# pkmtum/generative-physics-informed-pde

Measured on AMD Instinct MI355X. Metric: ELBO training-step samples/sec (64x64 grids), higher is better.
Workload: dtype f32; 1 GPU; BASELINE config 2/3: c64 grid, B_u=256 unlabeled + N_s=32 labeled per GPU, ROM 8x8, fused native step; global_batch=288, grid=64, parallelism=dp1, graph=True, graph_mode=streams, steps_per_replay=4, world=1, bn=replica

## Files before the change

generative-physics-informed-pde_amd/csrc/conv.hip:

```cpp
#include "common.h"
#include <stdlib.h>
#include <stdio.h>
#include <algorithm>
#include <string.h>
#include <string>
#include <type_traits>
#include <utility>
#include <vector>
#include <atomic>
#include <mutex>

using namespace gpi;

#pragma clang fp contract(on)

namespace {

constexpr int HALO = 4;

__device__ __attribute__((aligned(256))) float g_zero_page[64];

struct Div {
    uint32_t m, one;
};
// ... 1168 lines not shown
__host__ __device__ inline bool vop_op(const gpi_conv_desc& d) {
    return d.k == 5 && d.stride == 1 && !d.upsample && d.gin_off >= 0 && d.cin <= 4 && d.cout <= 2;
}
__host__ __device__ inline int bwd_rowlen(const gpi_conv_desc& d) {
    return d.cout * d.cin * d.k * d.k + (d.in_bn ? 2 * d.cin : 0);
}
__host__ __device__ inline int vop_mid_floats(int gh, int w_out, int rowlen, bool fuse);
template <bool B>
struct BoolC {
    static constexpr bool value = B;
};

template <int V>
struct IntC {
    static constexpr int value = V;
};

constexpr int GPI_BWD_WAVES = 6;
constexpr int SLAB_ROWS = 4;
__host__ __device__ inline int vop_mid_floats(int gh, int w_out, int rowlen, bool fuse) {
    return pad256(512 + SLAB_ROWS * rowlen);
}

constexpr int GPI_FUSE_WAVES = 5;
constexpr int GPI_FUSE_SHP_WAVES = 5;

template <typename T>
__device__ __forceinline__ T splat(float v);
template <>
__device__ __forceinline__ float splat<float>(float v) { return v; }
template <>
__device__ __forceinline__ f32x2 splat<f32x2>(float v) { return f32x2{v, v}; }

template <int K, int S, int UP, bool FUSE = false, bool HALF = false, int EXF = 0, int SHP = -1>
__global__ __launch_bounds__(256) __attribute__((amdgpu_waves_per_eu(K == 5 ? (FUSE ? (SHP >= 0 ? GPI_FUSE_SHP_WAVES : GPI_FUSE_WAVES) : 4) : GPI_BWD_WAVES))) void conv_bwd_kernel(gpi_conv_desc d, gpi_codec_ctx c, ConvGeom G) {
    fold_shape<SHP>(d, G);
    touch_kernargs<CONV_KARG_BYTES>();
    entry_signal(G);
    if (SKIP(G, 16)) return;
    ConvGeom Gt_;
    if constexpr (HALF) {
        const int lb0 = logical_block(G);
        const bool wgr0 = G.split && (G.xcd ? (lb0 & 1) != 0 : lb0 >= G.nblocks);
        const int tile0 = !G.split ? lb0 : (G.xcd ? lb0 >> 1 : (wgr0 ? lb0 - G.nblocks : lb0));
        Gt_ = G;
        if (tile0 >= G.nfull) set_half_tile(Gt_);
    }
    const ConvGeom& Gt = HALF ? Gt_ : G;
    constexpr int KK = K * K;
    extern __shared__ __attribute__((aligned(16))) float smem[];
    double* gst = (double*)smem;
    float* i_sc = smem + 8 * (d.cin + d.cout);
    float* i_sh = i_sc + d.cin;
    float* i_mean = i_sh + d.cin;
    float* i_inv = i_mean + d.cin;
    float* i_gam = i_inv + d.cin;
    float* o_coef = i_gam + d.cin;
    float* o_drop = o_coef + 4 * d.cout;
    const bool has_gin = d.gin_off >= 0;
    const bool obn = d.gout_mode == 0;
    const int KD = d.cout * KK;
    const int KD4 = (KD + 3) & ~3;
    const bool vop = FUSE || (K == 5 && S == 1 && !UP && has_gin && d.cin <= 4 && d.cout <= 2);
    const int J = d.cin * KK;
    const int rowlen = d.cout * J + (d.in_bn ? 2 * d.cin : 0);
    float* wD = smem + bwd_hdr(d.cin, d.cout);
    const int nwd = (has_gin && !vop) ? KD4 * 16 : 0;
    float* const mid = wD;
// ... 284 lines not shown
        constexpr bool bern = EXF == 2;
        using acc_t = std::conditional_t<bern, float, f32x2>;
        const float scl = karg_sel(c.loss_scale, T.grp);
        const float xlo = bern ? karg_sel(c.tgt_lo, T.grp) : 0.f;
        const int nrg = (Gt.gh + RPF - 1) / RPF, nitem = nrg * d.w_out;
        auto fwd_items = [&](auto ci_c) {
            constexpr int CIN = decltype(ci_c)::value;
            for (int it = tid; it < nitem; it += 256) {
                const int rg = dq(it, Gt.d_wout), x = it - rg * d.w_out;
                const int j0 = rg * RPF;
                float tv[bern ? 1 : RPF];
                uint32_t tb = tb0;
                if constexpr (bern) {
                    if (it != tid) {
                        tb = 0;
#pragma unroll
                        for (int p = 0; p < RPF; ++p) {
                            const int oy = gy0 + j0 + p;
                            const bool ok = j0 + p < Gt.gh && oy >= 0 && oy < d.h_out;
                            tb |= ((ok ? as_gld(tg)[oy * d.w_out + x] : 0.f) != xlo ? 1u : 0u) << p;
                        }
                    }
                } else {
#pragma unroll
                    for (int p = 0; p < RPF; ++p) {
                        const int oy = gy0 + j0 + p;
                        const bool ok = j0 + p < Gt.gh && oy >= 0 && oy < d.h_out;
                        tv[p] = it == tid ? tv0[p] : (ok ? as_gld(tg)[oy * d.w_out + x] : 0.f);
                    }
                }
                acc_t acc[RPF];
#pragma unroll
                for (int p = 0; p < RPF; ++p) acc[p] = splat<acc_t>(0.f);
#pragma unroll(bern ? 1 : CIN)
                for (int ci = 0; ci < CIN; ++ci) {
                    if (ci >= d.cin) break;
                    const float* acol = al + ci * Gt.rh * Gt.P + HALO + x - PADK;
#pragma unroll(bern ? 1 : K)
                    for (int kx = 0; kx < K; ++kx) {
                        float v[RPF + K - 1];
#pragma unroll
                        for (int r = 0; r < RPF + K - 1; ++r) v[r] = acol[min(j0 + r, Gt.rh - 1) * Gt.P + kx];
                        acc_t w[K];
#pragma unroll
                        for (int ky = 0; ky < K; ++ky) {
                            const int i = ((ci * K + kx) * K + ky) * NCO;
                            w[ky] = *reinterpret_cast<const acc_t*>(mid + 256 + i);
                        }
#pragma unroll
                        for (int r = 0; r < RPF + K - 1; ++r) {
#pragma unroll
                            for (int p = 0; p < RPF; ++p) {
                                const int ky = r - p;
                                if (ky < 0 || ky >= K) continue;
                                acc[p] = __builtin_elementwise_fma(w[ky], splat<acc_t>(v[r]), acc[p]);
                            }
                        }
                    }
                }
#pragma unroll
                for (int p = 0; p < RPF; ++p) {
                    const int j = j0 + p, oy = gy0 + j;
                    if (j >= Gt.gh || oy < 0 || oy >= d.h_out) continue;
                    const bool own = j >= PADK && j < PADK + Gt.th;
                    float* g0 = gl + j * Gt.PG + HALO + x;
                    if constexpr (bern) {
                        float ll, gv;
// ... 224 lines not shown
                                const int co2 = i2 / K, kx2 = i2 - co2 * K;
                                if (ucls) {
                                    const int ci2 = j2 >> 1, rr = j2 & 1, py = (T.oy0 + wv) & 1;
                                    const int kyl = rr ? 1 + py : 0, kyh = rr ? 2 : py;
                                    float* const sp = slab + co2 * J + ci2 * KK + kx2;
                                    sp[kyl * K] = acc[u][r];
                                    if (kyh != kyl) sp[kyh * K] = acc[u][r];
                                } else {
                                    const int ci2 = j2 / K, ky2 = j2 - ci2 * K;
                                    slab[co2 * J + ci2 * KK + ky2 * K + kx2] = acc[u][r];
                                }
                            }
                        }
                    }
                }
            }
        }
    };
    const int bsel = Gt.alt == 1 ? (int)(blockIdx.x >> 8) : Gt.alt == 2 ? (int)(blockIdx.x >> 3) : (int)blockIdx.x;
    const bool wg_late = FUSE && Gt.alt != 0 && (bsel & 1) != 0;
    if (vop && !wg_late) wgrad_phase();
    PHASE(5);

    float sd = 0.f, sdx = 0.f;
    if (nmblk > 0) {
        float l_bet = 0.f, l_rgam = 0.f, l_gam = 0.f;
        if (d.in_bn) {
            l_gam = i_gam[ci_l];
            l_bet = i_sh[ci_l] + i_mean[ci_l] * i_sc[ci_l];
            l_rgam = 1.f / l_gam;
        }
        const float* arow0 = alb + (ci_l * Gt.rh + (py0 - iy0)) * Gt.P + HALO;
        const int nkd = KD4 >> 2;
        for (int round = 0; wv + 16 * round < nmblk; ++round) {
            if (round > 0 && S != 2) own_load(round, pv4);
#pragma unroll
            for (int u = 0; u < 4; ++u) {
                const int m = wv + 4 * (4 * round + u);
                if (m < nmblk) {
                    const int i = 16 * m + l16;
                    const int qy = dq(i, Gt.d_win), px = i - qy * d.w_in;
                    f32x4 acc = {0.f, 0.f, 0.f, 0.f};
                    if (S == 2) {
                        const int nbc = nmblk >> 2, cls = m / nbc, mb = m - cls * nbc;
                        const int ry = cls >> 1, rx = cls & 1;
                        const int nky = (K - ((ry + d.pad) & 1) + 1) >> 1, nkx = (K - ((rx + d.pad) & 1) + 1) >> 1;
                        const int nk = __builtin_amdgcn_readfirstlane(d.cout * nky * nkx);
                        const int cp = 16 * mb + l16, a2 = dq(cp, Gt.d_w2), b2 = cp - a2 * (d.w_in >> 1);
                        const float* ab = gl + ((py0 >> 1) - gy0 + a2) * Gt.PG + b2 + HALO;
                        const int2* tAB = reinterpret_cast<const int2*>(ktab + cls * 2 * KD4);
                        const int nks = (nk + 3) >> 2;
                        int ks = 0;
                        for (; ks + 4 <= nks; ks += 4) {
                            int2 t[4];
                            float a[4], b[4];
#pragma unroll
                            for (int u = 0; u < 4; ++u) t[u] = tAB[4 * (ks + u) + kq];
#pragma unroll
                            for (int u = 0; u < 4; ++u) {
                                a[u] = ab[t[u].x];
                                b[u] = wD[t[u].y + l16];
                            }
#pragma unroll
                            for (int u = 0; u < 4; ++u) acc = mfma4(4 * (ks + u) + kq < nk ? a[u] : 0.f, b[u], acc);
                        }
                        for (; ks < nks; ++ks) {
// ... 278 lines not shown

size_t bwd_lds(const gpi_conv_desc& d, const ConvGeom& G) {
    return sizeof(float) * bwd_lds_floats(d, G.rh, G.P, G.gh, G.PG, G.zreg, G.fuse != 0);
}

bool lsum_op(const gpi_conv_desc& d, const ConvGeom& G) {
    static const int on = env_int("GPI_LSUM", 2);
    if (!on || vop_op(d) || G.fuse) return false;
    if ((on == 2 && d.h_out * d.w_out > 256) || (on == 3 && d.h_out * d.w_out > 64)) return false;
    if (d.k == 7 && d.stride == 2 && !d.upsample && d.cin == 1 && d.gin_off < 0 && d.cout <= 16) return false;
    if (d.cout * d.k > 32 || d.cin * d.k > 32) return false;
    const size_t avail = bwd_lds_floats(d, G.rh, G.P, G.gh, G.PG, G.zreg, false) - bwd_hdr(d.cin, d.cout);
    return avail >= (size_t)4 * bwd_rowlen(d);
}

bool vsum_op(const gpi_conv_desc& d, const ConvGeom& G) {
    static const int on = env_int("GPI_VSUM", 1);
    if (!on || !(d.k == 7 && d.stride == 2 && !d.upsample && d.cin == 1 && d.gin_off < 0 && d.cout <= 16)) return false;
    return (size_t)img_floats(d.cout, G.gh, G.PG) >= (size_t)4 * bwd_rowlen(d);
}

typedef void (*conv_kernel_t)(gpi_conv_desc, gpi_codec_ctx, ConvGeom);

#ifndef GPI_CONV_SHAPE_NOFOLD
#define GPI_CONV_SHAPE_NOFOLD {-1}
#endif
constexpr int kNoFold[] = GPI_CONV_SHAPE_NOFOLD;
constexpr bool no_fold(int i) {
    for (int v : kNoFold)
        if (v == i) return true;
    return false;
}

template <int I>
conv_kernel_t shape_kernel() {
    constexpr ShapeC s = kShapes[I];
    if constexpr (no_fold(I)) return nullptr;
    else if constexpr (s.fwd != 0) return conv_fwd_kernel<s.D_k, s.D_stride, s.D_upsample, s.cp, s.npxk, s.half != 0, I>;
    else return conv_bwd_kernel<s.D_k, s.D_stride, s.upk, s.fusek != 0, s.half != 0, s.exf, I>;
}

template <int LO, int... I>
conv_kernel_t shape_kernel_at(int i, std::integer_sequence<int, I...>) {
    static const conv_kernel_t t[] = {shape_kernel<LO + I>()..., nullptr};
    return t[i];
}

}

namespace gpi_conv_parts {
__attribute__((visibility("hidden"))) void* shape_part1(int i);
__attribute__((visibility("hidden"))) void* shape_part2(int i);
__attribute__((visibility("hidden"))) void* shape_part3(int i);
#if GPI_CONV_SHAPE_PART > 0
#define GPI_PART_FN_(p) shape_part##p
#define GPI_PART_FN(p) GPI_PART_FN_(p)
void* GPI_PART_FN(GPI_CONV_SHAPE_PART)(int i) {
    constexpr int lo = kBounds[GPI_CONV_SHAPE_PART], n = kBounds[GPI_CONV_SHAPE_PART + 1] - lo;
    return (void*)shape_kernel_at<lo>(i, std::make_integer_sequence<int, n>{});
}
#endif
}

namespace {
#if GPI_CONV_SHAPE_PART == 0

template <int K, int S, int UP, int NPX, bool HALF>
conv_kernel_t pick_cp_h(int cp) {
    if (cp == 2) return conv_fwd_kernel<K, S, UP, 2, NPX, HALF>;
    if (cp == 4) return conv_fwd_kernel<K, S, UP, 4, NPX, HALF>;
    if (cp == 6) return conv_fwd_kernel<K, S, UP, 6, NPX, HALF>;
    return conv_fwd_kernel<K, S, UP, 8, NPX, HALF>;
}

template <int K, int S, int UP, int NPX>
conv_kernel_t pick_cp(int cp, bool half = false) {
    if constexpr (NPX != 0) {
        if (half) return pick_cp_h<K, S, UP, NPX, true>(cp);
    }
    return pick_cp_h<K, S, UP, NPX, false>(cp);
}

template <int K, int S, int UP>
conv_kernel_t pick(int cp, bool fwd, int npx, bool half, bool ucls = false) {
    if constexpr (UP != 0) {
        if (!fwd && ucls) return half ? conv_bwd_kernel<K, S, 2, false, true> : conv_bwd_kernel<K, S, 2>;
    }
    if (!fwd) return half ? conv_bwd_kernel<K, S, UP, false, true> : conv_bwd_kernel<K, S, UP>;
    if constexpr (K == 3 && S == 1) {
        if (npx == NPX_ROWS2) {
            if (cp == 4) return half ? conv_fwd_kernel<K, S, UP, 4, NPX_ROWS2, true> : conv_fwd_kernel<K, S, UP, 4, NPX_ROWS2>;
            if (cp == 6) return half ? conv_fwd_kernel<K, S, UP, 6, NPX_ROWS2, true> : conv_fwd_kernel<K, S, UP, 6, NPX_ROWS2>;
            return half ? conv_fwd_kernel<K, S, UP, 8, NPX_ROWS2, true> : conv_fwd_kernel<K, S, UP, 8, NPX_ROWS2>;
        }
    }
// ... 59 lines not shown
    s.wout = d.wpart_off >= 0;
    s.ext_in = d.in_off < 0;
    if (fuse) {
        s.half = half;
        s.exf = exf;
        s.upk = 0;
    } else if (!fwd) {
        s.half = half;
        s.upk = (d.upsample && G.ucls) ? 2 : d.upsample;
    } else {
        const int npx = G.cg > 1 ? 0 : G.npx;
        s.npxk = (npx == 0 && !(d.upsample == 0 && d.k <= 3)) ? 1 : npx;
        s.half = s.npxk == 0 ? 0 : half;
        s.cp = cp;
    }
#define F(n) s.D_##n = d.n;
    SHAPE_D(F)
#undef F
#define F(n) s.G_##n = G.n;
    SHAPE_G(F)
#undef F
#define F(n) s.M_##n = (int)G.n.m, s.O_##n = (int)G.n.one;
    SHAPE_GD(F)
#undef F
#define F(n) s.A_##n = G.ha.n;
    SHAPE_A(F)
#undef F
#define F(n) s.AM_##n = (int)G.ha.n.m, s.AO_##n = (int)G.ha.n.one;
    SHAPE_AD(F)
#undef F
    return s;
}

conv_kernel_t shape_kernel_any(int i) {
    if (i < 0 || i >= kNumShapes) return nullptr;
    if (i < kBounds[1]) return shape_kernel_at<0>(i, std::make_integer_sequence<int, kBounds[1]>{});
    if (i < kBounds[2]) return (conv_kernel_t)gpi_conv_parts::shape_part1(i - kBounds[1]);
    if (i < kBounds[3]) return (conv_kernel_t)gpi_conv_parts::shape_part2(i - kBounds[2]);
    return (conv_kernel_t)gpi_conv_parts::shape_part3(i - kBounds[3]);
}

std::atomic<int64_t> g_shape_planned{0}, g_shape_matched{0};
std::vector<ShapeC> g_shapes_seen;
std::mutex g_shapes_mu;

int shape_index(const ShapeC& s) {
    for (int i = 0; i < kNumShapes; ++i)
        if (memcmp(&kShapes[i], &s, sizeof(ShapeC)) == 0) return i;
    return -1;
}

int launch(const gpi_conv_desc& d, const gpi_codec_ctx& c, hipStream_t st, bool fwd, bool fuse = false,
           uint32_t* sig = nullptr, const int64_t* sig_epoch = nullptr, bool dry = false) {
    ConvGeom G;
    if (!conv_geom(d, c.groups, G, fwd, fuse)) return GPI_ERR_UNSUPPORTED;
    if (sig && !sig_epoch) return GPI_ERR_ARG;
    G.sig = sig;
    G.sig_epoch = sig_epoch;
    const bool bern = d.epilogue == GPI_EPI_BERNOULLI_LOSS;
    if (bern && (d.cout != 1 || d.gout_mode != 1)) return GPI_ERR_ARG;
    if (bern && (d.k != 5 || d.stride != 1 || d.upsample)) return GPI_ERR_UNSUPPORTED;
    if (bern && (fwd || fuse) && !dry)
        for (int g = 0; g < c.groups.n_groups; ++g)
            if (!c.tgt[g]) return GPI_ERR_ARG;
    if (fuse && (fwd || d.k != 5 || d.stride != 1 || d.upsample || d.cout != (bern ? 1 : 2) || d.cin > 4 ||
                 d.drop_off >= 0 || d.gout_mode != 1 || d.gin_off < 0 || !loss_epi(d.epilogue)))
        return GPI_ERR_UNSUPPORTED;
    if (gauss_epi(d.epilogue) && d.cout != 2) return GPI_ERR_ARG;
    if (d.in_off < 0 && !c.ext_in) return GPI_ERR_ARG;
    if (!aligned_ok(d, c, fwd)) return GPI_ERR_UNSUPPORTED;
    if (!fwd && d.gin_off >= 0 && ((G.ph * d.w_in) & 15)) return GPI_ERR_UNSUPPORTED;
    if (!fwd && d.gin_off >= 0 && d.stride == 2 && ((d.w_in & 7) || (G.ph & 1))) return GPI_ERR_UNSUPPORTED;
    const int cp = cp_of(d);
    const int exf = bern ? 2 : d.epilogue == GPI_EPI_GAUSS_EXP_LOSS ? 1 : 0;
    conv_kernel_t k = select_kernel(d, cp, fwd, G.cg > 1 ? 0 : G.npx, G.nfull < G.nblocks, G.ucls != 0, fuse, exf);
    if (!k) return GPI_ERR_UNSUPPORTED;
    static const float* zero = nullptr;
    if (!zero && !dry) {
        void* p = nullptr;
        if (hipGetSymbolAddress(&p, HIP_SYMBOL(g_zero_page)) != hipSuccess) return GPI_ERR_LAUNCH;
        zero = (const float*)p;
    }
    G.zero = zero;
    if (!fwd) G.lsum = lsum_op(d, G) ? 1 : 0;
    if (!fwd) G.vsum = vsum_op(d, G) ? 1 : 0;
    const size_t lds = fwd ? fwd_lds(d, G, cp) : bwd_lds(d, G);
    if (lds > 160 * 1024) return GPI_ERR_UNSUPPORTED;
    if (!fwd && d.gin_off >= 0 && !fuse && !vop_op(d)) {
        static const int split_env = env_int("GPI_BWD_SPLIT", 1);
        const int per_cu = std::min((int)(160000 / std::max<size_t>(lds, 1)), d.k == 5 ? 4 : 6);
        G.split = (split_env && d.wpart_off >= 0 && 2 * G.nblocks <= std::min(per_cu, 4) * 256) ? 1 : 0;
    }
    const int grid = G.nblocks * (G.split ? 2 : 1);
    G.grid = grid;
    G.xcd = xcd_mode(fwd, fuse, G.split != 0, G.nfull < G.nblocks) ? 1 : 0;
    static const int fuse_alt = env_int("GPI_FUSE_ALT", 1);
    G.alt = fuse ? fuse_alt : 0;
    {
        const int shapes_on = env_int("GPI_CONV_SHAPES", 1);
        static const int record = env_int("GPI_CONV_SHAPES_RECORD", 0);
        const ShapeC s = shape_of(d, G, fwd, fuse, cp, exf);
        g_shape_planned += dry ? 0 : 1;
        const int si = shapes_on ? shape_index(s) : -1;
        const conv_kernel_t ks = si >= 0 ? shape_kernel_any(si) : nullptr;
        if (ks) {
            k = ks;
            g_shape_matched += dry ? 0 : 1;
        }
        if (record || dry) {
            std::lock_guard<std::mutex> lk(g_shapes_mu);
            bool seen = false;
            for (const ShapeC& q : g_shapes_seen) seen = seen || memcmp(&q, &s, sizeof(ShapeC)) == 0;
            if (!seen) g_shapes_seen.push_back(s);
        }
        if (dry) return GPI_OK;
    }
#ifdef GPI_PHASE_TIMING
    static const int dbg_print = env_int("GPI_DBG_PRINT", 0);
    if (dbg_print)
        fprintf(stderr, "conv %s k%d s%d up%d cin%d cout%d in%dx%d out%dx%d th%d blocks %d lds %zu\n",
                fwd ? "fwd" : "bwd", d.k, d.stride, d.upsample, d.cin, d.cout, d.h_in, d.w_in, d.h_out, d.w_out, G.th,
                G.nblocks, lds);
#endif
    if (lds > 64 * 1024) {
        if (hipFuncSetAttribute((const void*)k, hipFuncAttributeMaxDynamicSharedMemorySize, (int)lds) != hipSuccess)
            return GPI_ERR_LAUNCH;
    }
    hipLaunchKernelGGL(k, dim3(grid), dim3(256), lds, st, d, c, G);
    GPI_CHECK_LAUNCH();
    return GPI_OK;
}

#ifndef GPI_RROWS
#define GPI_RROWS 64
#endif
constexpr int RROWS = GPI_RROWS;

// ... 80 lines not shown
    const int threads = n_items * max_channels;
    hipLaunchKernelGGL(bn_running_kernel, dim3((threads + 255) / 256), dim3(256), 0, (hipStream_t)stream, items, n_items,
                       max_channels, stats, n_stats, momentum);
    GPI_CHECK_LAUNCH();
    return GPI_OK;
}

constexpr uint32_t PROBE_SENTINEL = 0xdeadbeefu;
__global__ __launch_bounds__(64) void buffer_lds_probe_kernel(const float* src, int bytes, const int32_t* off16,
                                                              const int32_t* off4, uint32_t* out) {
    __shared__ __attribute__((aligned(16))) float lds[320];
    const int lane = threadIdx.x;
    for (int i = lane; i < 320; i += 64) lds[i] = __builtin_bit_cast(float, PROBE_SENTINEL);
    __syncthreads();
    const rsrc_t rs = make_rsrc(src, bytes);
    blds16(rs, off16[lane], lds);
    blds4(rs, off4[lane], lds + 256);
    asm volatile("s_waitcnt vmcnt(0)" ::: "memory");
    __syncthreads();
    for (int i = lane; i < 320; i += 64) out[i] = __builtin_bit_cast(uint32_t, lds[i]);
}

extern "C" int gpi_debug_buffer_lds_probe(const float* src, int32_t bytes, const int32_t* off16, const int32_t* off4,
                                          uint32_t* out, void* stream) {
    if (!src || !off16 || !off4 || !out || bytes <= 0 || (bytes & 15) || ((uintptr_t)src & 15)) return GPI_ERR_ARG;
    hipLaunchKernelGGL(buffer_lds_probe_kernel, dim3(1), dim3(64), 0, (hipStream_t)stream, src, (int)bytes, off16, off4,
                       out);
    GPI_CHECK_LAUNCH();
    return GPI_OK;
}

#ifdef GPI_PHASE_TIMING
extern "C" int gpi_debug_phase_stamps(unsigned long long* phase, unsigned long long* rt) {
    static unsigned long long zeros[4096 * 16];
    if (hipMemcpyFromSymbol(phase, HIP_SYMBOL(g_phase), sizeof(zeros)) != hipSuccess) return GPI_ERR_LAUNCH;
    if (hipMemcpyFromSymbol(rt, HIP_SYMBOL(g_rt), sizeof(unsigned long long) * 4096 * 2) != hipSuccess)
        return GPI_ERR_LAUNCH;
    if (hipMemcpyToSymbol(HIP_SYMBOL(g_phase), zeros, sizeof(zeros)) != hipSuccess) return GPI_ERR_LAUNCH;
    if (hipMemcpyToSymbol(HIP_SYMBOL(g_rt), zeros, sizeof(unsigned long long) * 4096 * 2) != hipSuccess)
        return GPI_ERR_LAUNCH;
    return GPI_OK;
}
#endif

extern "C" int gpi_conv_blocks(const gpi_conv_desc* op, const gpi_groups* groups, int32_t* blocks) {
    if (!op || !groups || !blocks) return GPI_ERR_ARG;
    ConvGeom G;
    if (!conv_geom(*op, *groups, G, false)) return GPI_ERR_UNSUPPORTED;
    *blocks = G.nblocks * ((vop_op(*op) || lsum_op(*op, G) || vsum_op(*op, G)) ? 1 : SLAB_ROWS);
    return GPI_OK;
}

extern "C" int gpi_conv_launch_info(const gpi_conv_desc* op, const gpi_groups* groups, int fwd, int32_t* info) {
    if (!op || !groups || !info) return GPI_ERR_ARG;
    ConvGeom G;
    if (!conv_geom(*op, *groups, G, fwd != 0)) return GPI_ERR_UNSUPPORTED;
    const int cp = cp_of(*op);
    info[0] = G.th;
    info[1] = G.nblocks;
    info[2] = (int32_t)(fwd ? fwd_lds(*op, G, cp) : bwd_lds(*op, G));
    info[3] = cp;
    info[4] = G.npx;
    info[5] = G.P;
    info[6] = G.PG;
    return GPI_OK;
}

extern "C" int gpi_conv_shape_info(int64_t* info) {
    if (!info) return GPI_ERR_ARG;
    info[0] = kNumShapes;
    info[1] = g_shape_planned;
    info[2] = g_shape_matched;
    {
        std::lock_guard<std::mutex> lk(g_shapes_mu);
        info[3] = (int64_t)g_shapes_seen.size();
    }
    return GPI_OK;
}

extern "C" int gpi_conv_shape_plan(const gpi_conv_desc* op, const gpi_codec_ctx* ctx, int fwd, int fuse) {
    if (!op || !ctx) return GPI_ERR_ARG;
    return launch(*op, *ctx, nullptr, fwd != 0, fuse != 0, nullptr, nullptr, true);
}

extern "C" int gpi_conv_shapes_dump(char* buf, int64_t len) {
    if (!buf || len <= 0) return GPI_ERR_ARG;
    std::lock_guard<std::mutex> lk(g_shapes_mu);
    std::string out = "#define GPI_CONV_SHAPE_COUNT " + std::to_string(g_shapes_seen.size()) + "\n#define GPI_CONV_SHAPE_LIST";
    for (const ShapeC& s : g_shapes_seen) {
        const int* f = reinterpret_cast<const int*>(&s);
        out += " \\\n    {";
        for (size_t i = 0; i < sizeof(ShapeC) / sizeof(int); ++i) out += (i ? "," : "") + std::to_string(f[i]);
        out += "},";
    }
    out += "\n";
    if ((int64_t)out.size() + 1 > len) return GPI_ERR_ARG;
    memcpy(buf, out.c_str(), out.size() + 1);
    return GPI_OK;
}

extern "C" int gpi_conv_forward(const gpi_conv_desc* op, const gpi_codec_ctx* ctx, void* stream) {
    if (!op || !ctx) return GPI_ERR_ARG;
    return launch(*op, *ctx, (hipStream_t)stream, true);
}

extern "C" int gpi_conv_backward(const gpi_conv_desc* op, const gpi_codec_ctx* ctx, void* stream) {
    if (!op || !ctx) return GPI_ERR_ARG;
    return launch(*op, *ctx, (hipStream_t)stream, false);
}

// ... 73 lines not shown
```

generative-physics-informed-pde_amd/gpi/_lib.py:

```python
import ctypes as C
import os

import torch

HERE = os.path.dirname(os.path.abspath(__file__))
LIB_PATH = os.path.join(HERE, 'libgpi_hip.so')
if os.environ.get('GPI_LIB_VARIANT'):
    LIB_PATH = os.path.join(HERE, 'libgpi_hip_%s.so' % os.environ['GPI_LIB_VARIANT'])
if os.environ.get('GPI_PHASE_TIMING') == '1':
    LIB_PATH = os.path.join(HERE, 'libgpi_hip_timing%s.so' % (
        ('_' + os.environ['GPI_LIB_VARIANT']) if os.environ.get('GPI_LIB_VARIANT') else ''))

GPI_MAX_GROUPS = 4
GPI_MAX_CIN = 32
GPI_MAX_COUT = 8
GPI_MAX_REDUCE_ITEMS = 48
GPI_MAX_GEMM_ITEMS = 12
GPI_REPLICAS = int(os.environ.get('GPI_REPLICAS', '16'))
FINALIZE_ACCUMULATE = 1
FINALIZE_ZERO = 2

EPI_STORE, EPI_STORE_STATS, EPI_GAUSS_LOSS, EPI_GAUSS_EXP_LOSS, EPI_BERNOULLI_LOSS = 0, 1, 2, 3, 4
HEAD_ENC, HEAD_REPARAM, HEAD_QZ, HEAD_LATENT, HEAD_GP, HEAD_LOCKX = 0x01, 0x02, 0x04, 0x08, 0x10, 0x20
HEAD_PART_ENC, HEAD_PART_Q, HEAD_VALU = 0x100, 0x200, 0x400
# ... 197 lines not shown

GPI_MAX_DRAWS = 6
DRAW_RANDN, DRAW_DROPOUT, DRAW_SUBSET, DRAW_GAUSS = 0, 1, 2, 3


class DrawItem(C.Structure):
    _fields_ = [('kind', i32), ('p', f32), ('out', vp), ('n', i64), ('k', i64), ('sub', u64), ('seed', u64),
                ('mean', vp), ('logsigma', vp)]


GPI_MAX_RANKS = 16
GPI_BNX_MSG = 64
BNX_FOLD, BNX_UNFOLD, BNX_PEER = 0, 1, 2


class BnExchangeDesc(C.Structure):
    _fields_ = [('stats', vp), ('n_stats', i64), ('stat0', i32), ('n', i32), ('f0', i32), ('mode', i32),
                ('scale', vp), ('msg', vp), ('rank', i32), ('world', i32),
                ('peer_buf', vp * GPI_MAX_RANKS), ('peer_flag', vp * GPI_MAX_RANKS), ('seq', vp), ('err', vp)]


STRUCTS = [Stat, Groups, ConvDesc, CodecCtx, ReduceItem, HeadDesc, GemmItem, RomDesc, ResidualDesc, AdamDesc,
           VoQueryDesc, VoMomentsDesc, VoConditionDesc, VoPrecisionDesc, GpSampleDesc,
           VoGalerkinDesc, StepEpilogueDesc, FomDesc, RandomFieldDesc, VoSparse, DrawItem, BnExchangeDesc,
           BnEvalItem, VoEnergyDesc, RomFitDesc, GpMlpDesc, GpMlpSampleDesc]

SIGNATURES = {
    'gpi_version': (C.c_int, []),
    'gpi_replicas': (C.c_int, []),
    'gpi_source_sha': (C.c_char_p, []),
    'gpi_conv_shape_info': (C.c_int, [C.c_void_p]),
    'gpi_conv_shapes_dump': (C.c_int, [C.c_char_p, C.c_int64]),
    'gpi_conv_shape_plan': (C.c_int, [C.c_void_p, C.c_void_p, C.c_int, C.c_int]),
    'gpi_struct_sizes': (C.c_int, [C.POINTER(i64), C.c_int]),
    'gpi_error_string': (C.c_char_p, [C.c_int]),
    'gpi_conv_blocks': (C.c_int, [C.POINTER(ConvDesc), C.POINTER(Groups), C.POINTER(i32)]),
    'gpi_bn_running_update': (C.c_int, [vp, C.c_int, C.c_int, vp, i64, f32, vp]),
    'gpi_bn_eval_seed': (C.c_int, [vp, C.c_int, C.c_int, vp, i64, vp]),
    'gpi_affine': (C.c_int, [vp, vp, vp, vp, C.c_int, C.c_int, C.c_int, vp]),
    'gpi_conv_loss_fused': (C.c_int, [C.POINTER(ConvDesc), C.POINTER(CodecCtx), vp]),
    'gpi_conv_launch_info': (C.c_int, [C.POINTER(ConvDesc), C.POINTER(Groups), C.c_int, C.POINTER(i32)]),
    'gpi_conv_forward': (C.c_int, [C.POINTER(ConvDesc), C.POINTER(CodecCtx), vp]),
    'gpi_conv_backward': (C.c_int, [C.POINTER(ConvDesc), C.POINTER(CodecCtx), vp]),
    'gpi_codec_forward': (C.c_int, [C.POINTER(ConvDesc), C.c_int, C.POINTER(CodecCtx), vp]),
    'gpi_codec_backward': (C.c_int, [C.POINTER(ConvDesc), C.c_int, C.POINTER(CodecCtx), vp]),
    'gpi_conv_forward_sig': (C.c_int, [C.POINTER(ConvDesc), C.POINTER(CodecCtx), vp, vp, vp]),
    'gpi_conv_backward_sig': (C.c_int, [C.POINTER(ConvDesc), C.POINTER(CodecCtx), vp, vp, vp]),
    'gpi_codec_forward_sig': (C.c_int, [C.POINTER(ConvDesc), C.c_int, C.POINTER(CodecCtx), vp, vp, vp]),
    'gpi_codec_backward_sig': (C.c_int, [C.POINTER(ConvDesc), C.c_int, C.POINTER(CodecCtx), vp, vp, vp]),
    'gpi_wgrad_reduce': (C.c_int, [C.POINTER(ReduceItem), C.c_int, vp, vp, vp]),
    'gpi_head_forward': (C.c_int, [C.POINTER(HeadDesc), vp, vp, vp]),
    'gpi_head_backward': (C.c_int, [C.POINTER(HeadDesc), vp, vp, vp, vp]),
    'gpi_outer_gemm': (C.c_int, [C.POINTER(GemmItem), C.c_int, vp, vp, vp]),
    'gpi_rom': (C.c_int, [C.POINTER(RomDesc), vp]),
    'gpi_rom_fit': (C.c_int, [C.POINTER(RomFitDesc), vp]),
    'gpi_cgr_residual': (C.c_int, [C.POINTER(ResidualDesc), vp]),
    'gpi_grad_finalize': (C.c_int, [vp, vp, i64, C.c_int, vp, vp]),
    'gpi_adam': (C.c_int, [C.POINTER(AdamDesc), vp]),
    'gpi_step_epilogue': (C.c_int, [C.POINTER(StepEpilogueDesc), vp]),
    'gpi_step_epilogue_adam': (C.c_int, [C.POINTER(StepEpilogueDesc), C.POINTER(AdamDesc), vp, vp]),
    'gpi_fom_workspace': (i64, [i32]),
    'gpi_fom_solve': (C.c_int, [C.POINTER(FomDesc), vp]),
    'gpi_random_field': (C.c_int, [C.POINTER(RandomFieldDesc), vp]),
    'gpi_randn': (C.c_int, [vp, i64, u64, vp, u64, vp]),
    'gpi_draws': (C.c_int, [vp, C.c_int, vp, vp]),
    'gpi_bn_exchange': (C.c_int, [C.POINTER(BnExchangeDesc), vp]),
# ... 118 lines not shown
```

include/gpi.h:

```cpp
#ifndef GPI_H
#define GPI_H

#include <stdint.h>

#ifdef __cplusplus
extern "C" {
#endif

#define GPI_OK 0
#define GPI_ERR_ARG (-1)
#define GPI_ERR_LAUNCH (-2)
#define GPI_ERR_UNSUPPORTED (-3)

#define GPI_MAX_GROUPS 4
#define GPI_MAX_CIN 32
#define GPI_MAX_COUT 8
#define GPI_MAX_REDUCE_ITEMS 48
#define GPI_MAX_GEMM_ITEMS 12
#ifndef GPI_REPLICAS
#define GPI_REPLICAS 16
#endif
#ifndef GPI_EPILOGUE_MAX_WG
#define GPI_EPILOGUE_MAX_WG 512
#endif
// ... 333 lines not shown
int gpi_bn_eval_seed(const gpi_bn_eval_item* items, int n_items, int max_channels, gpi_stat* stats, int64_t n_stats,
                     void* stream);

int gpi_affine(const float* W, const float* b, const float* in, float* out, int rows, int d_out, int d_in,
               void* stream);

#define GPI_MAX_RANKS 16
#define GPI_BNX_MSG 64
#define GPI_BNX_FOLD   0
#define GPI_BNX_UNFOLD 1
#define GPI_BNX_PEER   2
typedef struct gpi_bn_exchange_desc {
    gpi_stat* stats;
    int64_t n_stats;
    int32_t stat0, n, f0, mode;
    const double* scale;
    double* msg;
    int32_t rank, world;
    double* peer_buf[GPI_MAX_RANKS];
    uint32_t* peer_flag[GPI_MAX_RANKS];
    uint32_t* seq;
    uint32_t* err;
} gpi_bn_exchange_desc;
int gpi_bn_exchange(const gpi_bn_exchange_desc* d, void* stream);
int gpi_peer_alloc(int64_t bytes, void** ptr, void* ipc_handle);
int gpi_peer_open(const void* ipc_handle, void** ptr);
int gpi_peer_close(void* ptr, int own);

int gpi_conv_blocks(const gpi_conv_desc* op, const gpi_groups* groups, int32_t* blocks);
int gpi_conv_launch_info(const gpi_conv_desc* op, const gpi_groups* groups, int fwd, int32_t* info);
int gpi_conv_shape_info(int64_t* info);
int gpi_conv_shape_plan(const gpi_conv_desc* op, const gpi_codec_ctx* ctx, int fwd, int fuse);
int gpi_conv_shapes_dump(char* buf, int64_t len);
int gpi_conv_forward(const gpi_conv_desc* op, const gpi_codec_ctx* ctx, void* stream);
int gpi_conv_backward(const gpi_conv_desc* op, const gpi_codec_ctx* ctx, void* stream);
int gpi_conv_loss_fused(const gpi_conv_desc* op, const gpi_codec_ctx* ctx, void* stream);
int gpi_codec_forward(const gpi_conv_desc* ops, int n_ops, const gpi_codec_ctx* ctx, void* stream);
int gpi_codec_backward(const gpi_conv_desc* ops, int n_ops, const gpi_codec_ctx* ctx, void* stream);
int gpi_conv_forward_sig(const gpi_conv_desc* op, const gpi_codec_ctx* ctx, uint32_t* flag, const int64_t* epoch,
                         void* stream);
int gpi_conv_backward_sig(const gpi_conv_desc* op, const gpi_codec_ctx* ctx, uint32_t* flag, const int64_t* epoch,
                          void* stream);
int gpi_codec_forward_sig(const gpi_conv_desc* ops, int n_ops, const gpi_codec_ctx* ctx, uint32_t* flag,
                          const int64_t* epoch, void* stream);
int gpi_codec_backward_sig(const gpi_conv_desc* ops, int n_ops, const gpi_codec_ctx* ctx, uint32_t* flag,
                           const int64_t* epoch, void* stream);
int gpi_wgrad_reduce(const gpi_reduce_item* items, int n_items, const float* wpart, double* gacc, void* stream);

int gpi_head_forward(const gpi_head_desc* d, const float* params, float* ws, void* stream);
int gpi_head_backward(const gpi_head_desc* d, const float* params, float* ws, double* gacc, void* stream);

int gpi_outer_gemm(const gpi_gemm_item* items, int n_items, const float* ws, double* gacc, void* stream);

int gpi_rom(const gpi_rom_desc* d, void* stream);
int gpi_rom_fit(const gpi_rom_fit_desc* d, void* stream);
int gpi_cgr_residual(const gpi_residual_desc* d, void* stream);

int gpi_vo_rows(int32_t n_fine, int32_t nc, int32_t flags);
int gpi_vo_query(const gpi_vo_query_desc* d, void* stream);
int gpi_vo_galerkin(const gpi_vo_galerkin_desc* d, void* stream);
int gpi_vo_moments(const gpi_vo_moments_desc* d, void* stream);
int gpi_vo_condition(const gpi_vo_condition_desc* d, void* stream);
int gpi_vo_pattern(const double* gamma, int32_t n, int32_t m, int32_t d_y, int32_t r, int32_t* rows, int32_t* count,
                   uint8_t* work, void* stream);
int gpi_vo_sparse_values(const double* gamma, int32_t n, int32_t m, int32_t d_y, const gpi_vo_sparse* sp,
                         void* stream);
// ... 151 lines not shown
```

Measured before the change: 673,000 samples/s.

## Add register-resident input-gradient block path for eligible backward conv shapes

Adds an IGB specialization of the backward conv kernel for eligible stride-1 shapes with small kernel-depth. It preloads kernel offsets and weight columns into registers and processes several 16-pixel blocks per wave with batched MFMA accumulation, replacing the generic per-block loop. Wave occupancy hints are derived from the shape's LDS footprint. The input-channel unroll in another loop is capped at 4. The change also reworks the phase-timing stamp collection across shape parts. Register pressure and the occupancy hints could reduce occupancy for some shapes.

```diff
diff --git a/generative-physics-informed-pde_amd/csrc/conv.hip b/generative-physics-informed-pde_amd/csrc/conv.hip
--- a/generative-physics-informed-pde_amd/csrc/conv.hip
+++ b/generative-physics-informed-pde_amd/csrc/conv.hip
@@ -1224,8 +1224,36 @@
 template <>
 __device__ __forceinline__ f32x2 splat<f32x2>(float v) { return f32x2{v, v}; }
 
-template <int K, int S, int UP, bool FUSE = false, bool HALF = false, int EXF = 0, int SHP = -1>
-__global__ __launch_bounds__(256) __attribute__((amdgpu_waves_per_eu(K == 5 ? (FUSE ? (SHP >= 0 ? GPI_FUSE_SHP_WAVES : GPI_FUSE_WAVES) : 4) : GPI_BWD_WAVES))) void conv_bwd_kernel(gpi_conv_desc d, gpi_codec_ctx c, ConvGeom G) {
+constexpr int GPI_IGB_MAX_STEPS = 18;
+constexpr bool igb_shape(const ShapeC& s) {
+    const int nkd = (s.D_cout * s.D_k * s.D_k + 3) >> 2;
+    const bool vop = s.D_k == 5 && s.D_stride == 1 && !s.D_upsample && s.D_cin <= 4 && s.D_cout <= 2;
+    const int blocks = (s.G_ph * s.D_w_in) >> 4;
+    const bool gains = blocks >= 16 || (s.D_upsample && blocks >= 8);
+    return !s.fwd && !s.fusek && s.has_gin && s.D_stride == 1 && !vop && nkd <= GPI_IGB_MAX_STEPS && gains;
+}
+constexpr int igb_pad(int n, int a) { return (n + a - 1) & ~(a - 1); }
+constexpr int igb_lds_bytes(const ShapeC& s) {
+    const int KD4 = (s.D_cout * s.D_k * s.D_k + 3) & ~3;
+    const int hdr = igb_pad(8 * (s.D_cin + s.D_cout) + 5 * s.D_cin + 5 * s.D_cout, 64);
+    const int gimg = igb_pad(4 * (s.D_cout * s.G_gh * (s.G_PG / 4) + IMG_MARGIN4), 256);
+    const int aimg = igb_pad(4 * (s.D_cin * s.G_rh * (s.G_P / 4) + IMG_MARGIN4), 256);
+    const bool zimg = s.D_gout_mode == 0 && !s.G_zreg;
+    return 4 * (hdr + igb_pad(KD4 * 16, 256) + igb_pad(KD4, 256) + gimg + (zimg ? gimg : 0) + aimg);
+}
+constexpr int igb_waves_of(int lds_bytes) {
+    const int n = 160000 / (lds_bytes > 0 ? lds_bytes : 1);
+    return n >= GPI_BWD_WAVES ? GPI_BWD_WAVES : n <= 4 ? 4 : n;
+}
+template <int K, bool FUSE, int SHP, bool IGB>
+constexpr int bwd_waves() {
+    if constexpr (IGB) return igb_waves_of(igb_lds_bytes(kShapes[SHP]));
+    return K == 5 ? (FUSE ? (SHP >= 0 ? GPI_FUSE_SHP_WAVES : GPI_FUSE_WAVES) : 4) : GPI_BWD_WAVES;
+}
+
+template <int K, int S, int UP, bool FUSE = false, bool HALF = false, int EXF = 0, int SHP = -1, bool IGB = false>
+__global__ __launch_bounds__(256) __attribute__((amdgpu_waves_per_eu(bwd_waves<K, FUSE, SHP, IGB>()))) void conv_bwd_kernel(gpi_conv_desc d, gpi_codec_ctx c, ConvGeom G) {
+    static_assert(!IGB || (SHP >= 0 && igb_shape(kShapes[SHP >= 0 ? SHP : kNumShapes])), "IGB: eligible shape entries only");
     fold_shape<SHP>(d, G);
     touch_kernargs<CONV_KARG_BYTES>();
     entry_signal(G);
@@ -1576,7 +1604,7 @@
                 acc_t acc[RPF];
 #pragma unroll
                 for (int p = 0; p < RPF; ++p) acc[p] = splat<acc_t>(0.f);
-#pragma unroll(bern ? 1 : CIN)
+#pragma unroll(bern ? 1 : 4)
                 for (int ci = 0; ci < CIN; ++ci) {
                     if (ci >= d.cin) break;
                     const float* acol = al + ci * Gt.rh * Gt.P + HALO + x - PADK;
@@ -1867,6 +1895,84 @@
         }
         const float* arow0 = alb + (ci_l * Gt.rh + (py0 - iy0)) * Gt.P + HALO;
         const int nkd = KD4 >> 2;
+        if constexpr (IGB) {
+            constexpr int NKD = (kShapes[SHP >= 0 ? SHP : kNumShapes].D_cout * KK + 3) >> 2;
+            constexpr int GS = UP ? 2 : 4;
+            int koff[NKD];
+            float wcol[NKD];
+#pragma unroll
+            for (int ks = 0; ks < NKD; ++ks) {
+                koff[ks] = ktab[4 * ks + kq];
+                wcol[ks] = wD[(4 * ks + kq) * 16 + l16];
+            }
+            auto blocks = [&](auto nl_c, int round) {
+                constexpr int NL = decltype(nl_c)::value;
+                const float* gp0[NL];
+                f32x4 acc[NL];
+#pragma unroll
+                for (int u = 0; u < NL; ++u) {
+                    const int i = 16 * (wv + 4 * (4 * round + u)) + l16;
+                    const int qy = dq(i, Gt.d_win), px = i - qy * d.w_in;
+                    gp0[u] = gl + (UP ? 2 * (qy * Gt.PG + px) : qy * Gt.PG + px);
+                    acc[u] = f32x4{0.f, 0.f, 0.f, 0.f};
+                }
+#pragma unroll
+                for (int ks0 = 0; ks0 < NKD; ks0 += GS) {
+                    float a[GS][NL];
+#pragma unroll
+                    for (int j = 0; j < GS; ++j) {
+                        if (ks0 + j >= NKD) break;
+#pragma unroll
+                        for (int u = 0; u < NL; ++u) {
+                            const float* ga = gp0[u] + koff[ks0 + j];
+                            a[j][u] = UP ? (ga[0] + ga[1]) + (ga[Gt.PG] + ga[Gt.PG + 1]) : ga[0];
+                        }
+                    }
+#pragma unroll
+                    for (int j = 0; j < GS; ++j) {
+                        if (ks0 + j >= NKD) break;
+#pragma unroll
+                        for (int u = 0; u < NL; ++u) acc[u] = mfma4(a[j][u], wcol[ks0 + j], acc[u]);
+                    }
+                }
+                if (cok) {
+#pragma unroll
+                    for (int u = 0; u < NL; ++u) {
+                        const int i0 = 16 * (wv + 4 * (4 * round + u)) + 4 * kq;
+                        float* gp = ws + gin_off + ibase + i0;
+                        const int qy0 = dq(i0, Gt.d_win), px0 = i0 - qy0 * d.w_in;
+                        const f32x4 av = *(const f32x4*)(arow0 + qy0 * Gt.P + px0);
+                        float o[4];
+#pragma unroll
+                        for (int q = 0; q < 4; ++q) {
+                            if (d.in_bn) {
+                                const float dbn = av[q] > 0.f ? acc[u][q] : 0.f;
+                                o[q] = pv4[u][q] + l_gam * dbn;
+                                sd += dbn;
+                                sdx += dbn * ((av[q] - l_bet) * l_rgam);
+                            } else {
+                                o[q] = pv4[u][q] + acc[u][q];
+                            }
+                        }
+                        st4(gp, f32x4{o[0], o[1], o[2], o[3]});
+                    }
+                }
+            };
+            const int nmb = (Gt.ph * d.w_in) >> 4;
+            const int nbw = (nmb & 3) == 0 ? nmb >> 2 : (nmb - wv + 3) >> 2;
+            int round = 0;
+            for (; 4 * round + 4 <= nbw; ++round) {
+                if (round > 0) own_load(round, pv4);
+                blocks(IntC<4>{}, round);
+            }
+            const int nl = nbw - 4 * round;
+            if (nl > 0) {
+                if (round > 0) own_load(round, pv4);
+                if (nl == 3) blocks(IntC<3>{}, round);
+                else if (nl == 2) blocks(IntC<2>{}, round);
+                else blocks(IntC<1>{}, round);
+            }
+        } else
         for (int round = 0; wv + 16 * round < nmblk; ++round) {
             if (round > 0 && S != 2) own_load(round, pv4);
 #pragma unroll
@@ -2211,35 +2317,60 @@
     return false;
 }
 
-template <int I>
+template <int I, bool IGB>
 conv_kernel_t shape_kernel() {
     constexpr ShapeC s = kShapes[I];
     if constexpr (no_fold(I)) return nullptr;
     else if constexpr (s.fwd != 0) return conv_fwd_kernel<s.D_k, s.D_stride, s.D_upsample, s.cp, s.npxk, s.half != 0, I>;
-    else return conv_bwd_kernel<s.D_k, s.D_stride, s.upk, s.fusek != 0, s.half != 0, s.exf, I>;
+    else return conv_bwd_kernel<s.D_k, s.D_stride, s.upk, s.fusek != 0, s.half != 0, s.exf, I, IGB && igb_shape(s)>;
 }
 
 template <int LO, int... I>
-conv_kernel_t shape_kernel_at(int i, std::integer_sequence<int, I...>) {
-    static const conv_kernel_t t[] = {shape_kernel<LO + I>()..., nullptr};
-    return t[i];
+conv_kernel_t shape_kernel_at(int i, bool igb, std::integer_sequence<int, I...>) {
+    static const conv_kernel_t t[] = {shape_kernel<LO + I, true>()..., nullptr};
+    static const conv_kernel_t t0[] = {shape_kernel<LO + I, false>()..., nullptr};
+    return igb ? t[i] : t0[i];
 }
 
 }
 
 namespace gpi_conv_parts {
-__attribute__((visibility("hidden"))) void* shape_part1(int i);
-__attribute__((visibility("hidden"))) void* shape_part2(int i);
-__attribute__((visibility("hidden"))) void* shape_part3(int i);
+__attribute__((visibility("hidden"))) void* shape_part1(int i, bool igb);
+__attribute__((visibility("hidden"))) void* shape_part2(int i, bool igb);
+__attribute__((visibility("hidden"))) void* shape_part3(int i, bool igb);
 #if GPI_CONV_SHAPE_PART > 0
 #define GPI_PART_FN_(p) shape_part##p
 #define GPI_PART_FN(p) GPI_PART_FN_(p)
-void* GPI_PART_FN(GPI_CONV_SHAPE_PART)(int i) {
+void* GPI_PART_FN(GPI_CONV_SHAPE_PART)(int i, bool igb) {
     constexpr int lo = kBounds[GPI_CONV_SHAPE_PART], n = kBounds[GPI_CONV_SHAPE_PART + 1] - lo;
-    return (void*)shape_kernel_at<lo>(i, std::make_integer_sequence<int, n>{});
+    return (void*)shape_kernel_at<lo>(i, igb, std::make_integer_sequence<int, n>{});
 }
 #endif
 }
+
+#ifdef GPI_PHASE_TIMING
+namespace gpi_conv_parts {
+__attribute__((visibility("hidden"))) int stamps_part0(unsigned long long* phase, unsigned long long* rt);
+__attribute__((visibility("hidden"))) int stamps_part1(unsigned long long* phase, unsigned long long* rt);
+__attribute__((visibility("hidden"))) int stamps_part2(unsigned long long* phase, unsigned long long* rt);
+__attribute__((visibility("hidden"))) int stamps_part3(unsigned long long* phase, unsigned long long* rt);
+#define GPI_STAMPS_FN_(p) stamps_part##p
+#define GPI_STAMPS_FN(p) GPI_STAMPS_FN_(p)
+int GPI_STAMPS_FN(GPI_CONV_SHAPE_PART)(unsigned long long* phase, unsigned long long* rt) {
+    constexpr size_t NP = 4096 * 16, NR = 4096 * 2;
+    static unsigned long long zeros[NP];
+    std::vector<unsigned long long> p(NP), r(NR);
+    if (hipMemcpyFromSymbol(p.data(), HIP_SYMBOL(g_phase), NP * sizeof(unsigned long long)) != hipSuccess ||
+        hipMemcpyFromSymbol(r.data(), HIP_SYMBOL(g_rt), NR * sizeof(unsigned long long)) != hipSuccess ||
+        hipMemcpyToSymbol(HIP_SYMBOL(g_phase), zeros, NP * sizeof(unsigned long long)) != hipSuccess ||
+        hipMemcpyToSymbol(HIP_SYMBOL(g_rt), zeros, NR * sizeof(unsigned long long)) != hipSuccess)
+        return GPI_ERR_LAUNCH;
+    for (size_t i = 0; i < NP; ++i) phase[i] += p[i];
+    for (size_t i = 0; i < NR; ++i) rt[i] += r[i];
+    return GPI_OK;
+}
+}
+#endif
 
 namespace {
 #if GPI_CONV_SHAPE_PART == 0
@@ -2365,12 +2496,12 @@
     return s;
 }
 
-conv_kernel_t shape_kernel_any(int i) {
+conv_kernel_t shape_kernel_any(int i, bool igb) {
     if (i < 0 || i >= kNumShapes) return nullptr;
-    if (i < kBounds[1]) return shape_kernel_at<0>(i, std::make_integer_sequence<int, kBounds[1]>{});
-    if (i < kBounds[2]) return (conv_kernel_t)gpi_conv_parts::shape_part1(i - kBounds[1]);
-    if (i < kBounds[3]) return (conv_kernel_t)gpi_conv_parts::shape_part2(i - kBounds[2]);
-    return (conv_kernel_t)gpi_conv_parts::shape_part3(i - kBounds[3]);
+    if (i < kBounds[1]) return shape_kernel_at<0>(i, igb, std::make_integer_sequence<int, kBounds[1]>{});
+    if (i < kBounds[2]) return (conv_kernel_t)gpi_conv_parts::shape_part1(i - kBounds[1], igb);
+    if (i < kBounds[3]) return (conv_kernel_t)gpi_conv_parts::shape_part2(i - kBounds[2], igb);
+    return (conv_kernel_t)gpi_conv_parts::shape_part3(i - kBounds[3], igb);
 }
 
 std::atomic<int64_t> g_shape_planned{0}, g_shape_matched{0};
@@ -2435,7 +2566,10 @@
         const ShapeC s = shape_of(d, G, fwd, fuse, cp, exf);
         g_shape_planned += dry ? 0 : 1;
         const int si = shapes_on ? shape_index(s) : -1;
-        const conv_kernel_t ks = si >= 0 ? shape_kernel_any(si) : nullptr;
+        const int ig_blocks = env_int("GPI_IG_BLOCKS", 1);
+        if (si >= 0 && ig_blocks && igb_shape(kShapes[si]) && igb_waves_of(igb_lds_bytes(kShapes[si])) != igb_waves_of((int)lds))
+            return GPI_ERR_LAUNCH;
+        const conv_kernel_t ks = si >= 0 ? shape_kernel_any(si, ig_blocks != 0) : nullptr;
         if (ks) {
             k = ks;
             g_shape_matched += dry ? 0 : 1;
@@ -2582,13 +2716,11 @@
 
 #ifdef GPI_PHASE_TIMING
 extern "C" int gpi_debug_phase_stamps(unsigned long long* phase, unsigned long long* rt) {
-    static unsigned long long zeros[4096 * 16];
-    if (hipMemcpyFromSymbol(phase, HIP_SYMBOL(g_phase), sizeof(zeros)) != hipSuccess) return GPI_ERR_LAUNCH;
-    if (hipMemcpyFromSymbol(rt, HIP_SYMBOL(g_rt), sizeof(unsigned long long) * 4096 * 2) != hipSuccess)
-        return GPI_ERR_LAUNCH;
-    if (hipMemcpyToSymbol(HIP_SYMBOL(g_phase), zeros, sizeof(zeros)) != hipSuccess) return GPI_ERR_LAUNCH;
-    if (hipMemcpyToSymbol(HIP_SYMBOL(g_rt), zeros, sizeof(unsigned long long) * 4096 * 2) != hipSuccess)
-        return GPI_ERR_LAUNCH;
+    memset(phase, 0, sizeof(unsigned long long) * 4096 * 16);
+    memset(rt, 0, sizeof(unsigned long long) * 4096 * 2);
+    for (auto part : {gpi_conv_parts::stamps_part0, gpi_conv_parts::stamps_part1, gpi_conv_parts::stamps_part2,
+                      gpi_conv_parts::stamps_part3})
+        if (const int rc = part(phase, rt)) return rc;
     return GPI_OK;
 }
 #endif
@@ -2626,6 +2758,11 @@
         info[3] = (int64_t)g_shapes_seen.size();
     }
     return GPI_OK;
+}
+
+extern "C" int gpi_conv_shape_igb(int index) {
+    if (index < 0 || index >= kNumShapes) return -1;
+    return !no_fold(index) && igb_shape(kShapes[index]) ? 1 : 0;
 }
 
 extern "C" int gpi_conv_shape_plan(const gpi_conv_desc* op, const gpi_codec_ctx* ctx, int fwd, int fuse) {
diff --git a/generative-physics-informed-pde_amd/gpi/_lib.py b/generative-physics-informed-pde_amd/gpi/_lib.py
--- a/generative-physics-informed-pde_amd/gpi/_lib.py
+++ b/generative-physics-informed-pde_amd/gpi/_lib.py
@@ -253,6 +253,7 @@
     'gpi_conv_shape_info': (C.c_int, [C.c_void_p]),
     'gpi_conv_shapes_dump': (C.c_int, [C.c_char_p, C.c_int64]),
     'gpi_conv_shape_plan': (C.c_int, [C.c_void_p, C.c_void_p, C.c_int, C.c_int]),
+    'gpi_conv_shape_igb': (C.c_int, [C.c_int]),
     'gpi_struct_sizes': (C.c_int, [C.POINTER(i64), C.c_int]),
     'gpi_error_string': (C.c_char_p, [C.c_int]),
     'gpi_conv_blocks': (C.c_int, [C.POINTER(ConvDesc), C.POINTER(Groups), C.POINTER(i32)]),
diff --git a/include/gpi.h b/include/gpi.h
--- a/include/gpi.h
+++ b/include/gpi.h
@@ -389,6 +389,7 @@
 int gpi_conv_shape_info(int64_t* info);
 int gpi_conv_shape_plan(const gpi_conv_desc* op, const gpi_codec_ctx* ctx, int fwd, int fuse);
 int gpi_conv_shapes_dump(char* buf, int64_t len);
+int gpi_conv_shape_igb(int index);
 int gpi_conv_forward(const gpi_conv_desc* op, const gpi_codec_ctx* ctx, void* stream);
 int gpi_conv_backward(const gpi_conv_desc* op, const gpi_codec_ctx* ctx, void* stream);
 int gpi_conv_loss_fused(const gpi_conv_desc* op, const gpi_codec_ctx* ctx, void* stream);
```

After: 675,800 samples/s, median of 6. Within noise of the previous version (+0.4%).
